# Fahad021/DER-VET

Hardware: AMD Instinct MI355X
Metric: dispatch LP windows/sec (whole node, 8760h monthly windows); % HBM roofline (higher is better)
Workload: dtype f64

## Files before the change

### der-vet_amd/csrc/dvh_band.hip

```cpp
#include <stdio.h>
#include <stdlib.h>

#include <algorithm>
#include <type_traits>

#include "dvh_device.h"

namespace dvh {
namespace {

constexpr int kBandSteps = 768;
constexpr int kJMax = 4;
constexpr int kNeedsEll = -2;

__host__ __device__ constexpr size_t band_lds_doubles(int B, int S, bool ice, bool lc) {
  const int NW = B / kWave, NC = ice ? 5 : 3, NR = ice ? 4 : 2;
  const size_t SB = (size_t)S * B;
  return 2 * (size_t)(B + 1) + kJMax + (size_t)kNRed * (NW + 1) + 4 + (size_t)kJMax * B + (NC + NR) * SB +
         (lc ? 5 * SB : 0) + (ice ? 6 * SB : 0);
}
__host__ __device__ constexpr size_t band_ints_bytes(int B, int S) { return sizeof(int32_t) * (4 * (size_t)S * B + 4); }
__host__ __device__ constexpr size_t band_drow_bytes(int B, int S) { return align16(sizeof(int32_t) * (size_t)S * B); }
__host__ __device__ constexpr size_t band_lds_bytes(int B, int S, bool ice, bool lc) {
  const size_t d = align16(sizeof(double) * band_lds_doubles(B, S, ice, lc));
  return (lc ? d : d + align16(band_ints_bytes(B, S))) + band_drow_bytes(B, S);
}
static_assert(band_lds_bytes(kBandSteps / 3, 3, false, true) == 77328, "three-step battery form: two windows per CU");
static_assert(band_lds_bytes(kBandSteps, 1, false, false) == 84192, "one-step battery form");
static_assert(band_lds_bytes(kBandSteps, 1, true, false) == 145632, "ICE form");

template <bool ICE>
struct BandTune {
  static constexpr bool kkt_inline = !ICE;
  static constexpr bool kkt_prefetch = !ICE;
  static constexpr bool pin_kx = ICE;
  static constexpr bool uniform_check_scalars = ICE;
  static constexpr bool gate_rdx = !ICE;
};
constexpr int kTauWavePrio = 2;

struct ColKkt {
  double rd2, cx, bt;
};
struct ColKktX : ColKkt {
  double rdx;
};
__device__ __noinline__ ColKkt col_kkt_o(double kt, double cj, double loj, double hij, double xj, float fd) {
  const double id = (double)__builtin_amdgcn_rcpf(fd);
  const double rs = cj - kt;
  const bool fl = isfinite(loj), fh = isfinite(hij);
  const double lam = (fl && fh) ? rs : (fl ? fmax(rs, 0.0) : (fh ? fmin(rs, 0.0) : 0.0));
  const double rd = (rs - lam) * id;
  return {rd * rd, cj * xj, (fl ? loj * fmax(lam, 0.0) : 0.0) + (fh ? hij * fmin(lam, 0.0) : 0.0)};
}
__device__ __forceinline__ ColKktX col_kkt_x_i(double kt, double cj, double loj, double hij, double xj, float fd) {
  const double id = (double)__builtin_amdgcn_rcpf(fd);
  const double rs = cj - kt;
  const bool fl = isfinite(loj), fh = isfinite(hij);
  const double lam = (fl && fh) ? rs : (fl ? fmax(rs, 0.0) : (fh ? fmin(rs, 0.0) : 0.0));
  const double rd = (rs - lam) * id;
  ColKktX r;
  r.rd2 = rd * rd;
  r.cx = cj * xj;
  r.bt = (fl ? loj * fmax(lam, 0.0) : 0.0) + (fh ? hij * fmin(lam, 0.0) : 0.0);
  r.rdx = fabs(rd) * fabs(xj * (double)fd);
  return r;
}
struct RowKkt {
  double rp2, y2;
};
__device__ __forceinline__ RowKkt row_kkt_i(double kv, double qi, double yi, float fd, int ge) {
  const double dr = (double)fd, idr = (double)__builtin_amdgcn_rcpf(fd);
  double r = (qi - kv) * idr;
  if (ge) r = fmax(r, 0.0);
  return {r * r, (yi * dr) * (yi * dr)};
}
__device__ __noinline__ RowKkt row_kkt_o(double kv, double qi, double yi, float fd, int ge) {
  return row_kkt_i(kv, qi, yi, fd, ge);
}
template <bool INL>
__device__ __forceinline__ RowKkt row_kkt_fn(double kv, double qi, double yi, float fd, int ge) {
  if constexpr (INL) return row_kkt_i(kv, qi, yi, fd, ge);
  else return row_kkt_o(kv, qi, yi, fd, ge);
}

constexpr int kNeedsPlain = -3;
#ifndef DVH_BAND_PROBE
#define DVH_BAND_PROBE 0
#endif
__device__ __forceinline__ unsigned long long probe_clock() {
#if DVH_BAND_PROBE
  return __builtin_amdgcn_s_memtime();
#else
  return 0ull;
#endif
}
__device__ __forceinline__ double fma_clamp01(double a, double b, double c) {
  double r;
  asm("v_fma_f64 %0, %1, %2, %3 clamp" : "=v"(r) : "v"(a), "v"(b), "v"(c));
  return r;
}

template <bool ICE>
__device__ __forceinline__ double usc(double v) {
  return BandTune<ICE>::uniform_check_scalars ? uniform(v) : v;
}
template <bool ICE>
__device__ __forceinline__ double sgpr_fresh(double v) {
  if constexpr (BandTune<ICE>::uniform_check_scalars) asm volatile("" : "+s"(v));
  return v;
}
template <int B, int S, bool ICE, bool LC, int WPS, bool GATE, bool BOX>
__device__ __forceinline__ void band_window(const Batch& b, const Work& w, const Chunk& ch, const Opts& o, const int k_in,
                                            const int tid) {
  const int k = __builtin_amdgcn_readfirstlane(k_in);
  using Tune = BandTune<ICE>;
  constexpr int NW = B / kWave;
  constexpr int SB = S * B;
  constexpr int NC = ICE ? 5 : 3;
  constexpr int NR = ICE ? 4 : 2;
  extern __shared__ __attribute__((aligned(16))) unsigned char smem[];
  const int kl = k - ch.first;
  const WinOff W = uniform_win(win_offsets(b, ch, k));
  const int n = W.n, m = W.m, meq = W.meq;
  const int lane = tid & 63, wid = __builtin_amdgcn_readfirstlane(tid >> 6);
  double* scal = w.scal + (int64_t)kl * kScal;
  const int T = meq - 1, J = n - (ICE ? 5 : 3) * T, MI = m - meq;
  const int MD = ICE ? MI - 2 * T : MI;
  auto bail = [&]() {
    if (tid == 0) {
      b.istats[2 * k] = kNeedsEll;
      b.istats[2 * k + 1] = 0;
    }
  };
  if (n > kSmallMax || m > kSmallMax || T < 1 || T > SB || J < 0 || J > kJMax || MD < 0 || MD > T ||
      (J == 0 && MD > 0)) {
    bail();
    return;
  }
  const int CE = 3 * T + J, CO = 4 * T + J;
  double* XE = reinterpret_cast<double*>(smem);
  double* YS = XE + (B + 1);
  double* XT = YS + (B + 1);
  double* red = XT + kJMax;
  double* TP = red + kNRed * (NW + 1) + 4;
  double* XP = TP + kJMax * B;
  double* YP = XP + NC * SB;
  double* RO = YP + NR * SB;
  double* CQ = RO + (ICE ? 6 * SB : 0);
  static_assert(sizeof(double) * (NC + NR) * SB >= band_ints_bytes(B, S), "the ints fit the images");
  int32_t* dcm = LC ? reinterpret_cast<int32_t*>(XP)
                    : reinterpret_cast<int32_t*>(smem + align16(sizeof(double) * band_lds_doubles(B, S, ICE, LC)));
  int32_t* ice_a = dcm + SB;
  int32_t* ice_b = ice_a + SB;
  int32_t* ice_n = ice_b + SB;
  int32_t* flag = ice_n + SB;
  int32_t* DRL = reinterpret_cast<int32_t*>(smem + band_lds_bytes(B, S, ICE, LC) - band_drow_bytes(B, S));

  const int32_t* gkp = b.indptr + W.row;
  const int32_t* gkc = b.indices + W.nz;
  const double* gkv = b.data + W.nz;
  const double* craw = b.c + W.on;
  const double* lraw = b.l + W.on;
  const double* uraw = b.u + W.on;
  const double* qraw = b.q + W.om;
  double* dcv = w.dc + W.wn;
  double* drv = w.dr + W.wm;
  auto dcf = [&](int j) -> double { return dcv[j]; };
  auto drf = [&](int i) -> double { return drv[i]; };
  double* xo_g = b.x + W.on;
  double* yo_g = b.y + W.om;

  for (int u = tid; u < SB; u += B) {
    dcm[u] = -1;
    ice_a[u] = 0x7fffffff;
    ice_b[u] = -1;
    ice_n[u] = 0;
  }
  if (tid == 0) flag[0] = flag[1] = flag[2] = 0;
  __syncthreads();
  int bad = 0, crossed = 0, unboxed = 0;
  for (int j = tid; j < J; j += B) crossed |= lraw[3 * T + j] > uraw[3 * T + j];
  for (int r = tid; r <= T; r += B) {
    const int p0 = gkp[r], len = gkp[r + 1] - p0;
    if (r == 0) {
      bad |= !(len == 1 && gkc[p0] == 2 * T);
      continue;
    }
    const int t = r - 1;
    if (len != (r < T ? 4 : 3)) {
      bad = 1;
      continue;
    }
    unsigned seen = 0;
    for (int e = 0; e < len; ++e) {
      const int c = gkc[p0 + e];
      const int kind = c == t ? 0 : c == T + t ? 1 : c == 2 * T + t ? 2 : (r < T && c == 2 * T + t + 1) ? 3 : 4;
      if (kind == 4 || ((seen >> kind) & 1u)) bad = 1;
      seen |= 1u << kind;
    }
    bad |= lraw[t] != 0.0 || lraw[T + t] != 0.0;
    crossed |= lraw[t] > uraw[t] || lraw[T + t] > uraw[T + t] || lraw[2 * T + t] > uraw[2 * T + t];
    if (BOX) unboxed |= !(isfinite(uraw[t]) && isfinite(uraw[T + t]) && isfinite(lraw[2 * T + t]) && isfinite(uraw[2 * T + t]));
    if (ICE) {
      if (BOX) unboxed |= !(isfinite(uraw[CE + t]) && isfinite(uraw[CO + t]));
      bad |= lraw[CE + t] != 0.0 || lraw[CO + t] != 0.0;
      crossed |= lraw[CE + t] > uraw[CE + t] || lraw[CO + t] > uraw[CO + t];
    }
  }
  for (int i = meq + tid; i < m; i += B) {
    const int p0 = gkp[i], len = gkp[i + 1] - p0;
    if (ICE && len == 2) {
      int te = -1, to = -1;
      for (int e = 0; e < 2; ++e) {
        const int c = gkc[p0 + e];
        if (c >= CE && c < CE + T) te = c - CE;
        else if (c >= CO && c < CO + T) to = c - CO;
      }
      if (te < 0 || te != to) {
        bad = 1;
        continue;
      }
      atomicMin(&ice_a[te], i);
      atomicMax(&ice_b[te], i);
      atomicAdd(&ice_n[te], 1);
      continue;
    }
    if (len != (ICE ? 4 : 3)) {
      bad = 1;
      continue;
    }
    int tc = -1, td = -1, jj = -1, te = ICE ? -1 : -2;
    for (int e = 0; e < len; ++e) {
      const int c = gkc[p0 + e];
      if (c < T) {
        bad |= tc >= 0;
        tc = c;
      } else if (c < 2 * T) {
        bad |= td >= 0;
        td = c - T;
      } else if (c >= 3 * T && c < 3 * T + J) {
        bad |= jj >= 0;
        jj = c - 3 * T;
      } else if (ICE && c >= CE && c < CE + T) {
        bad |= te >= 0;
        te = c - CE;
      } else {
        bad = 1;
      }
    }
    if (tc < 0 || td != tc || jj < 0 || (ICE && te != tc)) {
      bad = 1;
      continue;
    }
    if (atomicCAS(&dcm[tc], -1, i * 8 + jj) != -1) bad = 1;
  }
  if (bad) flag[0] = 1;
  if (crossed) flag[1] = 1;
  if (unboxed) flag[2] = 1;
  __syncthreads();
  if (ICE)
    for (int u = tid; u < T; u += B)
      if (ice_n[u] != 2) flag[0] = 1;
  __syncthreads();
  if (flag[1] != 0) {
    if (tid == 0) {
      scal[0] = 0.0;
      scal[6] = 3.0;
      b.istats[2 * k] = 1;
      b.istats[2 * k + 1] = 0;
      for (int u = 0; u < 4; ++u) b.stats[4 * k + u] = u == 0 ? NAN : 0.0;
    }
    return;
  }
  if (flag[0] != 0) {
    bail();
    return;
  }
  auto bail_plain = [&]() {
    if (tid == 0) {
      b.istats[2 * k] = kNeedsPlain;
      b.istats[2 * k + 1] = 0;
    }
  };
  if (BOX && flag[2] != 0) {
    bail_plain();
    return;
  }

  const int t0 = S * tid;
  bool val[S];
  double x[S][NC], xa[S][NC], cc[S][3], hi[S][3];
  double loe[S];
  double ks[S][4];
  double kd[S][4];
  double ka[S][2], kb[S][2];
  double kp0 = 0.0;
  double y[S][NR], ya[S][NR], q[S][2];
  int drow[S], jt[S], ra[S], rb[S];
  auto col = [&](int s, int v) { return v < 3 ? v * T + t0 + s : (v == 3 ? CE : CO) + t0 + s; };
  auto ro = [&](int u, int s) -> double& { return RO[(u * S + s) * B + tid]; };
  auto cqa = [&](int u, int s) -> double& { return CQ[(u * S + s) * B + tid]; };
#pragma unroll
  for (int s = 0; s < S; ++s) {
    const int t = t0 + s;
    val[s] = t < T;
#pragma unroll
    for (int v = 0; v < NC; ++v) x[s][v] = xa[s][v] = 0.0;
#pragma unroll
    for (int v = 0; v < 3; ++v) cc[s][v] = hi[s][v] = 0.0;
#pragma unroll
    for (int r = 0; r < NR; ++r) y[s][r] = ya[s][r] = 0.0;
#pragma unroll
    for (int u = 0; u < 4; ++u) ks[s][u] = kd[s][u] = 0.0;
    ka[s][0] = ka[s][1] = kb[s][0] = kb[s][1] = 0.0;
    q[s][0] = q[s][1] = 0.0;
    loe[s] = 0.0;
    drow[s] = -1;
    DRL[s * B + tid] = -1;
    jt[s] = 0;
    ra[s] = rb[s] = -1;
    if (ICE)
      for (int u = 0; u < 6; ++u) ro(u, s) = 0.0;
    if (LC)
      for (int u = 0; u < 5; ++u) cqa(u, s) = 0.0;
  }
  auto cof = [&](int s, int v) -> double { return v < 3 ? (LC ? cqa(v, s) : cc[s][v]) : ro(v - 3, s); };
  auto qv = [&](int s, int r) -> double { return LC ? cqa(3 + r, s) : q[s][r]; };
  auto hib = [&](int s, int v) -> double { return v < 3 ? hi[s][v] : ro(v - 1, s); };
  auto rhs = [&](int s, int r) -> double { return r < 2 ? qv(s, r) : ro(r + 2, s); };
#pragma unroll
  for (int s = 0; s < S; ++s) {
    if (!val[s]) continue;
    const int t = t0 + s;
    for (int p = gkp[t + 1]; p < gkp[t + 2]; ++p) {
      const int c = gkc[p];
      const double a = gkv[p];
      if (c == t) ks[s][0] = a;
      else if (c == T + t) ks[s][1] = a;
      else if (c == 2 * T + t) ks[s][2] = a;
      else ks[s][3] = a;
    }
    if (s == 0)
      for (int p = gkp[t]; p < gkp[t + 1]; ++p)
        if (gkc[p] == 2 * T + t) kp0 = gkv[p];
    const int dv = dcm[t];
    if (dv >= 0) {
      drow[s] = dv >> 3;
      DRL[s * B + tid] = drow[s];
      jt[s] = dv & 7;
      for (int p = gkp[drow[s]]; p < gkp[drow[s] + 1]; ++p) {
        const int c = gkc[p];
        const double a = gkv[p];
        if (c < T) kd[s][0] = a;
        else if (c < 2 * T) kd[s][1] = a;
        else if (c < 3 * T + J) kd[s][2] = a;
        else kd[s][3] = a;
      }
    }
    if (ICE) {
      ra[s] = ice_a[t];
      rb[s] = ice_b[t];
      for (int p = gkp[ra[s]]; p < gkp[ra[s] + 1]; ++p) (gkc[p] < CO ? ka[s][0] : ka[s][1]) = gkv[p];
      for (int p = gkp[rb[s]]; p < gkp[rb[s] + 1]; ++p) (gkc[p] < CO ? kb[s][0] : kb[s][1]) = gkv[p];
    }
  }
  auto row_of = [&](int s, int r) -> int {
    return r == 0 ? (val[s] ? t0 + s + 1 : -1) : r == 1 ? drow[s] : (val[s] ? (r == 2 ? ra[s] : rb[s]) : -1);
  };
  constexpr int kInitLane = kWave - 1;
  static_assert(kJMax < kInitLane, "tau lanes and the init-row lane are distinct");
  const bool tlane = wid == 0 && lane < J, ilane = wid == 0 && lane == kInitLane;
  double sp[6] = {0.0, 0.0, 0.0, 0.0, 0.0, 0.0};

  double fcv[S][NC], frv[S][NR], fsp = 1.0, kin0 = 0.0;
#pragma unroll
  for (int s = 0; s < S; ++s) {
#pragma unroll
    for (int v = 0; v < NC; ++v) fcv[s][v] = 1.0;
#pragma unroll
    for (int r = 0; r < NR; ++r) frv[s][r] = 1.0;
  }
  if (ilane) kin0 = gkv[gkp[0]];
  auto factor = [](double a) { return a > 0.0 ? __builtin_amdgcn_rsq(a) : 1.0; };
  auto exchange = [&]() {
    XE[tid] = fcv[0][2];
    YS[tid + 1] = frv[S - 1][0];
    if (tid == 0) XE[B] = 1.0;
    if (tid < kJMax) XT[tid] = tlane ? fsp : 1.0;
    if (ilane) YS[0] = fsp;
  };
  for (int pass = 0; pass <= o.ruiz_iters; ++pass) {
    const bool pc = pass == o.ruiz_iters;
    auto acc = [pc](double a, double v) { return pc ? a + v : fmax(a, v); };
    exchange();
    __syncthreads();
    const double fen = XE[tid + 1], frp = YS[tid];
    double nr[S][NR], nc[S][NC];
#pragma unroll
    for (int s = 0; s < S; ++s) {
      const double fe1 = s < S - 1 ? fcv[s < S - 1 ? s + 1 : s][2] : fen;
      const double rp = s == 0 ? frp : frv[s > 0 ? s - 1 : 0][0];
      const double kpr = s == 0 ? kp0 : ks[s > 0 ? s - 1 : 0][3];
      const double r0 = frv[s][0], r1 = frv[s][1], ftj = XT[jt[s]];
      nr[s][0] = acc(acc(acc(fabs(ks[s][0]) * r0 * fcv[s][0], fabs(ks[s][1]) * r0 * fcv[s][1]),
                         fabs(ks[s][2]) * r0 * fcv[s][2]),
                     fabs(ks[s][3]) * r0 * fe1);
      nr[s][1] = acc(acc(fabs(kd[s][0]) * r1 * fcv[s][0], fabs(kd[s][1]) * r1 * fcv[s][1]), fabs(kd[s][2]) * r1 * ftj);
      nc[s][0] = acc(fabs(ks[s][0]) * r0 * fcv[s][0], fabs(kd[s][0]) * r1 * fcv[s][0]);
      nc[s][1] = acc(fabs(ks[s][1]) * r0 * fcv[s][1], fabs(kd[s][1]) * r1 * fcv[s][1]);
      nc[s][2] = acc(fabs(kpr) * rp * fcv[s][2], fabs(ks[s][2]) * r0 * fcv[s][2]);
      if constexpr (ICE) {
        const double r2 = frv[s][NR > 2 ? 2 : 0], r3 = frv[s][NR > 3 ? 3 : 0];
        const double f3 = fcv[s][NC > 3 ? 3 : 0], f4 = fcv[s][NC > 4 ? 4 : 0];
        nr[s][1] = acc(nr[s][1], fabs(kd[s][3]) * r1 * f3);
        nr[s][NR > 2 ? 2 : 0] = acc(fabs(ka[s][0]) * r2 * f3, fabs(ka[s][1]) * r2 * f4);
        nr[s][NR > 3 ? 3 : 0] = acc(fabs(kb[s][0]) * r3 * f3, fabs(kb[s][1]) * r3 * f4);
        nc[s][NC > 3 ? 3 : 0] = acc(acc(fabs(kd[s][3]) * r1 * f3, fabs(ka[s][0]) * r2 * f3), fabs(kb[s][0]) * r3 * f3);
        nc[s][NC > 4 ? 4 : 0] = acc(fabs(ka[s][1]) * r2 * f4, fabs(kb[s][1]) * r3 * f4);
      }
    }
    for (int j = 0; j < J; ++j) {
      const double ftj = XT[j];
      double a = 0.0;
#pragma unroll
      for (int s = 0; s < S; ++s)
        if (jt[s] == j) a = acc(a, fabs(kd[s][2]) * frv[s][1] * ftj);
      TP[j * B + tid] = a;
    }
    double nsp = 0.0;
    if (ilane) nsp = fabs(kin0) * fsp * XE[0];
    __syncthreads();
    if (wid == 0) {
      for (int j = 0; j < J; ++j) {
        double a = TP[j * B + lane];
#pragma unroll
        for (int r = 1; r < NW; ++r) a = acc(a, TP[j * B + r * kWave + lane]);
        a = uniform(pc ? wave_sum_dpp(a) : wave_max(a));
        if (lane == j) nsp = a;
      }
    }
#pragma unroll
    for (int s = 0; s < S; ++s) {
#pragma unroll
      for (int v = 0; v < NC; ++v) fcv[s][v] *= factor(nc[s][v]);
#pragma unroll
      for (int r = 0; r < NR; ++r) frv[s][r] *= factor(nr[s][r]);
    }
    if (tlane || ilane) fsp *= factor(nsp);
    __syncthreads();
  }
  {
    auto oor = [](double f) { return !(f >= 0x1p-100 && f <= 0x1p100); };
    bool out = oor(fsp);
#pragma unroll
    for (int s = 0; s < S; ++s) {
#pragma unroll
      for (int v = 0; v < NC; ++v) out |= oor(fcv[s][v]);
#pragma unroll
      for (int r = 0; r < NR; ++r) out |= oor(frv[s][r]);
    }
    if (__syncthreads_or(out)) {
      bail();
      return;
    }
  }
  exchange();
  __syncthreads();
  {
    const double fen = XE[tid + 1], frp = YS[tid];
    kp0 = kp0 * frp * fcv[0][2];
#pragma unroll
    for (int s = 0; s < S; ++s) {
      const double fe1 = s < S - 1 ? fcv[s < S - 1 ? s + 1 : s][2] : fen;
      const double r0 = frv[s][0], r1 = frv[s][1];
      ks[s][0] = ks[s][0] * r0 * fcv[s][0];
      ks[s][1] = ks[s][1] * r0 * fcv[s][1];
      ks[s][2] = ks[s][2] * r0 * fcv[s][2];
      ks[s][3] = ks[s][3] * r0 * fe1;
      kd[s][0] = kd[s][0] * r1 * fcv[s][0];
      kd[s][1] = kd[s][1] * r1 * fcv[s][1];
      kd[s][2] = kd[s][2] * r1 * XT[jt[s]];
      if constexpr (ICE) {
        const double r2 = frv[s][NR > 2 ? 2 : 0], r3 = frv[s][NR > 3 ? 3 : 0];
        const double f3 = fcv[s][NC > 3 ? 3 : 0], f4 = fcv[s][NC > 4 ? 4 : 0];
        kd[s][3] = kd[s][3] * r1 * f3;
        ka[s][0] = ka[s][0] * r2 * f3;
        ka[s][1] = ka[s][1] * r2 * f4;
        kb[s][0] = kb[s][0] * r3 * f3;
        kb[s][1] = kb[s][1] * r3 * f4;
      }
    }
    if (ilane) kin0 = kin0 * fsp * XE[0];
  }
  double nrm[4] = {0.0, 0.0, 0.0, 0.0};
#pragma unroll
  for (int s = 0; s < S; ++s) {
    if (!val[s]) continue;
    const int t = t0 + s;
#pragma unroll
    for (int v = 0; v < NC; ++v) {
      const int j = col(s, v);
      const double d = fcv[s][v], cj = craw[j];
      const double csj = cj * d, lsj = lraw[j] / d, usj = uraw[j] / d;
      if (v < 3) {
        hi[s][v] = usj;
        if (LC)
          cqa(v, s) = csj;
        else
          cc[s][v] = csj;
      } else {
        ro(v - 1, s) = usj;
        ro(v - 3, s) = csj;
      }
      if (v == 2) loe[s] = lsj;
      x[s][v] = xa[s][v] = fmin(fmax(o.warm ? xo_g[j] / d : 0.0, lsj), usj);
      nrm[0] += csj * csj;
      nrm[2] += cj * cj;
      dcv[j] = d;
      w.fc[W.wn + j] = (float)d;
    }
#pragma unroll
    for (int r = 0; r < NR; ++r) {
      const int i = row_of(s, r);
      if (i < 0) continue;
      const double d = frv[s][r], qi = qraw[i], qsi = qi * d;
      if (r == 0) {
        if (LC)
          cqa(3, s) = qsi;
        else
          q[s][0] = qsi;
      } else if (r == 1) {
        if (LC)
          cqa(4, s) = qsi;
        else
          q[s][1] = qsi;
      } else {
        ro(r + 2, s) = qsi;
      }
      if (o.warm) y[s][r] = ya[s][r] = r == 0 ? yo_g[i] / d : fmax(yo_g[i] / d, 0.0);
      nrm[1] += qsi * qsi;
      nrm[3] += qi * qi;
      drv[i] = d;
      w.fr[W.wm + i] = (float)d;
    }
  }
  if (tlane) {
    const int j = 3 * T + lane;
    const double cj = craw[j], l0 = lraw[j] / fsp, h0 = uraw[j] / fsp;
    sp[0] = sp[1] = sp[5] = fmin(fmax(o.warm ? xo_g[j] / fsp : 0.0, l0), h0);
    sp[2] = cj * fsp;
    sp[3] = l0;
    sp[4] = h0;
    nrm[0] += sp[2] * sp[2];
    nrm[2] += cj * cj;
    dcv[j] = fsp;
    w.fc[W.wn + j] = (float)fsp;
  }
  if (ilane) {
    const double q0 = qraw[0];
    sp[3] = q0 * fsp;
    sp[4] = kin0;
    if (o.warm) sp[0] = sp[1] = sp[2] = yo_g[0] / fsp;
    nrm[1] += sp[3] * sp[3];
    nrm[3] += q0 * q0;
    drv[0] = fsp;
    w.fr[W.wm] = (float)fsp;
  }
  block_sum<B, 4>(nrm, red);
  const double ncs = sqrt(nrm[0]), nqs = sqrt(nrm[1]);
  const double pw0 = (ncs > 1e-10 && nqs > 1e-10) ? ncs / nqs : 1.0;
  int xta[S];
#pragma unroll
  for (int s = 0; s < S; ++s) xta[s] = lds_addr(XT + jt[s]);
  if constexpr (LC) __syncthreads();
  auto xpi = [&](int v, int s) -> double& { return XP[(v * S + s) * B + tid]; };
  auto ypi = [&](int r, int s) -> double& { return YP[(r * S + s) * B + tid]; };
  if (tid < kJMax) XT[tid] = 0.0;
  if (tid == 0) XE[B] = YS[B] = 0.0;
  XE[tid] = YS[tid] = 0.0;
  for (int u = tid; u < kJMax * B; u += B) TP[u] = 0.0;
#pragma unroll
  for (int s = 0; s < S; ++s) {
#pragma unroll
    for (int v = 0; v < NC; ++v) xpi(v, s) = x[s][v];
#pragma unroll
    for (int r = 0; r < NR; ++r) ypi(r, s) = y[s][r];
  }
  __syncthreads();

  auto kpv = [&](int s) { return s == 0 ? kp0 : ks[s > 0 ? s - 1 : 0][3]; };
  auto ktr = [&](int s, const double (&vr)[NR], double vprev, double (&out)[NC]) {
    out[0] = fma(kd[s][0], vr[1], ks[s][0] * vr[0]);
    out[1] = fma(kd[s][1], vr[1], ks[s][1] * vr[0]);
    out[2] = fma(ks[s][2], vr[0], kpv(s) * vprev);
    if constexpr (ICE) {
      out[3] = fma(kb[s][0], vr[3], fma(ka[s][0], vr[2], kd[s][3] * vr[1]));
      out[4] = fma(kb[s][1], vr[3], ka[s][1] * vr[2]);
    }
  };
  auto kown = [&](int s, const double (&v)[NC], double (&os)[NR]) {
    os[0] = fma(ks[s][2], v[2], fma(ks[s][1], v[1], ks[s][0] * v[0]));
    os[1] = fma(kd[s][1], v[1], kd[s][0] * v[0]);
    if constexpr (ICE) {
      os[1] = fma(kd[s][3], v[3], os[1]);
      os[2] = fma(ka[s][1], v[4], ka[s][0] * v[3]);
      os[3] = fma(kb[s][1], v[4], kb[s][0] * v[3]);
    }
  };
  auto kfin_next = [&](int s, double (&os)[NR], double vnext) { os[0] = fma(ks[s][3], vnext, os[0]); };
  auto kfin_tau = [&](int s, double (&os)[NR]) { os[1] = fma(kd[s][2], lds_ld(xta[s]), os[1]); };
  auto ktr_c = [&](int s, const double (&vr)[NR], double vprev, double (&out)[NC]) {
    out[0] = fma(kd[s][0], vr[1], fma(ks[s][0], vr[0], -cof(s, 0)));
    out[1] = fma(kd[s][1], vr[1], fma(ks[s][1], vr[0], -cof(s, 1)));
    out[2] = fma(ks[s][2], vr[0], fma(kpv(s), vprev, -cof(s, 2)));
    if constexpr (ICE) {
      out[3] = fma(kb[s][0], vr[3], fma(ka[s][0], vr[2], fma(kd[s][3], vr[1], -cof(s, 3))));
      out[4] = fma(kb[s][1], vr[3], fma(ka[s][1], vr[2], -cof(s, 4)));
    }
  };
  auto kown_q = [&](int s, const double (&v)[NC], double (&os)[NR]) {
    os[0] = fma(ks[s][2], v[2], fma(ks[s][1], v[1], fma(ks[s][0], v[0], -qv(s, 0))));
    os[1] = fma(kd[s][1], v[1], fma(kd[s][0], v[0], -qv(s, 1)));
    if constexpr (ICE) {
      os[1] = fma(kd[s][3], v[3], os[1]);
      os[2] = fma(ka[s][1], v[4], fma(ka[s][0], v[3], -rhs(s, 2)));
      os[3] = fma(kb[s][1], v[4], fma(kb[s][0], v[3], -rhs(s, 3)));
    }
  };
  auto tau_parts = [&](const double (&vd)[S]) {
    if (J == 1) {
      double a = kd[0][2] * vd[0];
#pragma unroll
      for (int s = 1; s < S; ++s) a = fma(kd[s][2], vd[s], a);
      TP[tid] = a;
    } else {
      for (int j = 0; j < J; ++j) {
        double a = (jt[0] == j ? kd[0][2] : 0.0) * vd[0];
#pragma unroll
        for (int s = 1; s < S; ++s) a = fma(jt[s] == j ? kd[s][2] : 0.0, vd[s], a);
        TP[j * B + tid] = a;
      }
    }
  };
  auto tau_parts_of = [&](const double (&vr)[S][NR]) {
    double vd[S];
#pragma unroll
    for (int s = 0; s < S; ++s) vd[s] = vr[s][1];
    tau_parts(vd);
  };
  auto tau_kt = [&]() {
    double res = 0.0;
// ... 10 lines not shown
  double eta = o.step_safety;
  if (o.power_iters > 0) {
    const int P = o.power_iters;
    const double v0 = 1.0 / sqrt((double)n);
    double vc[S][NC];
#pragma unroll
    for (int s = 0; s < S; ++s)
#pragma unroll
      for (int v = 0; v < NC; ++v) vc[s][v] = val[s] ? v0 : 0.0;
    double vtau = (wid == 0 && lane < J) ? v0 : 0.0;
    double nv[2] = {0.0, 0.0};
    double wr[S][NR];
#pragma unroll
    for (int s = 0; s < S; ++s)
#pragma unroll
      for (int r = 0; r < NR; ++r) wr[s][r] = 0.0;
    for (int pi = 0; pi <= P; ++pi) {
      if (pi > 0) {
        const double ysp = YS[tid];
#pragma unroll
        for (int s = 0; s < S; ++s) ktr(s, wr[s], s == 0 ? ysp : wr[s > 0 ? s - 1 : 0][0], vc[s]);
        if (wid == 0) {
          const double kt = tau_kt();
          vtau = lane < J ? kt : 0.0;
        }
      }
      if (pi >= P - 1) {
        double a = vtau * vtau;
#pragma unroll
        for (int s = 0; s < S; ++s)
#pragma unroll
          for (int v = 0; v < NC; ++v) a = fma(vc[s][v], vc[s][v], a);
        nv[pi - (P - 1)] = a;
      }
      if (pi == P) break;
      XE[tid] = vc[0][2];
      if (wid == 0 && lane < J) XT[lane] = vtau;
      __syncthreads();
      const double xen = XE[tid + 1];
#pragma unroll
      for (int s = 0; s < S; ++s) {
        kown(s, vc[s], wr[s]);
        kfin_next(s, wr[s], s == S - 1 ? xen : vc[s < S - 1 ? s + 1 : s][2]);
        kfin_tau(s, wr[s]);
      }
      YS[tid + 1] = wr[S - 1][0];
      if (ilane) YS[0] = sp[4] * XE[0];
      tau_parts_of(wr);
      __syncthreads();
    }
    block_sum<B, 2>(nv, red);
    if (nv[0] > 0.0 && nv[1] > 0.0) eta = o.step_safety / sqrt(sqrt(nv[1] / nv[0]));
    YS[tid] = 0.0;
    if (tid == 0) YS[B] = 0.0;
    for (int u = tid; u < kJMax * B; u += B) TP[u] = 0.0;
    __syncthreads();
  }
  if (o.warm) {
    YS[tid + 1] = y[S - 1][0];
    if (ilane) YS[0] = sp[0];
    if (J > 0) tau_parts_of(y);
    __syncthreads();
  }
  eta = uniform(eta);
  double pwi = pw0;
  if (o.warm) {
    double nv[2] = {0.0, 0.0};
#pragma unroll
    for (int s = 0; s < S; ++s) {
#pragma unroll
      for (int v = 0; v < NC; ++v) nv[0] += x[s][v] * x[s][v];
#pragma unroll
      for (int r = 0; r < NR; ++r) nv[1] += y[s][r] * y[s][r];
    }
    if (tlane) nv[0] += sp[0] * sp[0];
    if (ilane) nv[1] += sp[0] * sp[0];
    block_sum<B, 2>(nv, red);
    if (nv[0] > 1e-20 && nv[1] > 1e-20) {
      const double ratio = sqrt(nv[1] / nv[0]);
      pwi = sqrt(ratio * pw0);
    }
  }
  double pw = uniform(pwi);
  double tj[S][3];
  double cbox = 0.0;
  if constexpr (BOX) {
    double wb[S][NC];
    bool unb = false;
#pragma unroll
    for (int s = 0; s < S; ++s) {
#pragma unroll
      for (int v = 0; v < NC; ++v) {
        double wv = hib(s, v) - (v == 2 ? loe[s] : 0.0);
        unb |= !isfinite(wv);
        if (!(wv >= 0x1p-500)) wv = 0.0;
        wb[s][v] = wv;
      }
    }
    if (__syncthreads_or(unb)) {
      bail_plain();
      return;
    }
    XP[tid] = wb[0][2];
    XP[B + 1 + tid] = loe[0];
    if (tid == 0) XP[B] = XP[2 * B + 1] = 0.0;
    __syncthreads();
    const double wnx = XP[tid + 1], lnx = XP[B + 2 + tid], we0 = XP[0], le0 = XP[B + 1];
    __syncthreads();
    double cl[1] = {0.0};
    kp0 *= wb[0][2];
#pragma unroll
    for (int s = 0; s < S; ++s) {
      const double wn1 = s < S - 1 ? wb[s < S - 1 ? s + 1 : s][2] : wnx;
      const double ln1 = s < S - 1 ? loe[s < S - 1 ? s + 1 : s] : lnx;
      if (val[s]) {
        const double qs = fma(-ks[s][3], ln1, fma(-ks[s][2], loe[s], qv(s, 0)));
        if (LC)
          cqa(3, s) = qs;
        else
          q[s][0] = qs;
        cl[0] = fma(cof(s, 2), loe[s], cl[0]);
      }
      ks[s][0] *= wb[s][0];
      ks[s][1] *= wb[s][1];
      ks[s][2] *= wb[s][2];
      ks[s][3] *= wn1;
      kd[s][0] *= wb[s][0];
      kd[s][1] *= wb[s][1];
      if constexpr (ICE) {
        const double we = wb[s][NC > 3 ? 3 : 0], wo = wb[s][NC > 4 ? 4 : 0];
        kd[s][3] *= we;
        ka[s][0] *= we;
        ka[s][1] *= wo;
        kb[s][0] *= we;
        kb[s][1] *= wo;
      }
#pragma unroll
      for (int v = 0; v < NC; ++v) {
        const double lo = v == 2 ? loe[s] : 0.0, wv = wb[s][v], cs = cof(s, v) * wv;
        if (v >= 3)
          ro(v - 3, s) = cs;
        else if (LC)
          cqa(v, s) = cs;
        else
          cc[s][v] = cs;
        const double xv = wv > 0.0 ? fmin(fmax((x[s][v] - lo) / wv, 0.0), 1.0) : 0.0;
        x[s][v] = xa[s][v] = xv;
        xpi(v, s) = xv;
        if (v < 3)
          tj[s][v < 3 ? v : 0] = wv > 0.0 ? uniform(eta / pw) / (wv * wv) : 0.0;
        else
          ro(v - 1, s) = wv > 0.0 ? uniform(eta / pw) / (wv * wv) : 0.0;
      }
    }
    if (ilane) {
      sp[3] = fma(-sp[4], le0, sp[3]);
      sp[4] *= we0;
    }
    block_sum<B, 1>(cl, red);
    cbox = cl[0];
  }
  const double cnorm = uniform(sqrt(nrm[2])), qnorm = uniform(sqrt(nrm[3])), c0 = uniform(b.c0[k] + cbox);
  int it = 0, kin = 0, status = kIterLimit;
  double r0 = -1.0, rprev = -1.0;
  double* fin = red + kNRed * NW;
  if (tid == 0)
// ... 139 lines not shown
      }
      XE[tid] = xb[0][2];
#pragma unroll
      for (int s = 0; s < S; ++s) {
        kown_q(s, xb[s], kx[s]);
        if (s < S - 1) kfin_next(s, kx[s], xb[s < S - 1 ? s + 1 : s][2]);
      }
      if constexpr (W0) {
        tau_update(uniform(wave_sum_dpp(ta0 + ta1)), ca, cb, chk_tag);
      } else {
        if (wid == 0 && J > 1) tau_update(tau_kt(), ca, cb, chk_tag);
      }
    }
    pstamp(0);
    if constexpr (!W0 && Tune::pin_kx) {
#pragma unroll
      for (int s = 0; s < S; ++s)
#pragma unroll
        for (int r = 0; r < NR; ++r) asm volatile("" ::"v"(kx[s][r]));
    }
    lds_barrier();
    if constexpr (W0) __builtin_amdgcn_s_setprio(0);
    pstamp(1);
    {
      const double xen = XE[tid + 1];
      double xtv[S];
#pragma unroll
      for (int s = 0; s < S; ++s) xtv[s] = lds_ld(xta[s]);
      kfin_next(S - 1, kx[S - 1], xen);
#pragma unroll
      for (int s = 0; s < S; ++s) {
        kx[s][1] = fma(kd[s][2], xtv[s], kx[s][1]);
#pragma unroll
        for (int r = 1; r < ((ICE && !W0) ? 2 : NR); ++r) row_step(s, r);
      }
      if (J > 0) tau_parts_of(y);
#pragma unroll
      for (int s = !W0 ? S - 1 : 0; s < S; ++s) row_step(s, 0);
      YS[tid + 1] = y[S - 1][0];
      if (W0 || wid == 0) {
        if (ilane) {
          const double y0 = sp[0], ya0 = sp[1];
          const double q1 = fma(sigma, sp[3] - sp[4] * XE[0], y0);
          if (CHECK) {
            const double d = y0 - q1, da = q1 - ya0;
            mv2 += d * d;
            mv3 += da * da;
            sp[2] = q1;
          }
          const double yn = fma(ca, fma(2.0, q1, -y0), cb * ya0);
          sp[0] = yn;
          YS[0] = yn;
        }
      }
    }
    ++it;
    ++kin;
    pstamp(2);
    if constexpr (W0) {
#pragma unroll
      for (int s = 0; s < S; ++s) {
#pragma unroll
        for (int v = 0; v < NC; ++v) asm volatile("" ::"v"(x[s][v]));
#pragma unroll
        for (int r = 0; r < NR; ++r) asm volatile("" ::"v"(y[s][r]));
      }
    }
    lds_barrier();
    if constexpr (!W0) {
#pragma unroll
      for (int s = 0; s < S - 1; ++s) row_step(s, 0);
    }
    if constexpr (ICE && !W0) {
#pragma unroll
      for (int s = 0; s < S; ++s)
#pragma unroll
        for (int r = 2; r < NR; ++r) row_step(s, r);
    }
    pstamp(3);
  };

  using F = std::integral_constant<bool, false>;
  using Tt = std::integral_constant<bool, true>;
  pstamp(-1);
  while (it < o.max_iters) {
    if (--ck != 0) {
      if (w0)
        iterate(F(), Tt());
      else
        iterate(F(), F());
      continue;
    }
    ck = chk;
    if (w0)
      iterate(Tt(), Tt());
    else
      iterate(Tt(), F());
    const bool last = it + chk > o.max_iters;
    bool kkt = (--kk_ == 0) || last;
    if (kkt) kk_ = kkt_every;
    static_assert(kRdx == kNRed - 1, "the dual-residual term is the last reduced value");
    constexpr int NRED = Tune::gate_rdx ? kNRed : kNRed - 1;
    double acc[NRED];
    acc[0] = fma(tau_bs, mvb0, mv0);
    acc[1] = fma(tau_bs, mvb1, mv1);
    acc[2] = mv2;
    acc[3] = mv3;
#pragma unroll
    for (int u = 4; u < NRED; ++u) acc[u] = 0.0;
    double r = 0.0;
    if constexpr (GATE) {
      double acc4[4] = {acc[0], acc[1], acc[2], acc[3]};
      block_sum1<B, 4, true>(acc4, red);
#pragma unroll
      for (int u = 0; u < 4; ++u) acc[u] = acc4[u];
      r = usc<ICE>(sqrt(pw * acc[0] + acc[2] / pw));
      if (kkt && !last && kkt_gate_skip(o, gate, r)) {
        kkt = false;
        ++gate.skip;
      }
    }
    if (kkt) {
      float fcl[S][NC], frl[S][NR], fspl = 1.0f;
      if constexpr (Tune::kkt_prefetch) {
        const int to = S * opaque(tid);
        const float* fcw = w.fc + W.wn;
        const float* frw = w.fr + W.wm;
#pragma unroll
        for (int s = 0; s < S; ++s) {
          const bool vs = to + s < T;
#pragma unroll
          for (int v = 0; v < NC; ++v) {
            const int j = v < 3 ? v * T + to + s : (v == 3 ? CE : CO) + to + s;
            const float f = fcw[vs ? j : 0];
            fcl[s][v] = vs ? f : 1.0f;
          }
#pragma unroll
          for (int r = 0; r < NR; ++r) {
            const int i = r == 0 ? (vs ? to + s + 1 : -1) : r == 1 ? DRL[s * B + tid] : (vs ? (r == 2 ? ra[s] : rb[s]) : -1);
            const float f = frw[i >= 0 ? i : 0];
            frl[s][r] = i >= 0 ? f : 1.0f;
          }
        }
        const int lo_ = (to / S) & (kWave - 1);
        const float ft = fcw[tlane ? 3 * T + lo_ : 0], fi = frw[0];
        fspl = tlane ? ft : ilane ? fi : 1.0f;
      }
      double xp[S][NC], yp[S][NR];
      load_images(xp, yp);
      XE[tid] = xp[0][2];
      YS[tid + 1] = yp[S - 1][0];
      if (ilane) YS[0] = sp[2];
      if (tlane) XT[lane] = sp[5];
      if (J > 0) tau_parts_of(yp);
      lds_barrier();
      auto col_kkt = [&](int j, double kt, double cj, double loj, double hij, double xj, float fpre) {
        const float fd = Tune::kkt_prefetch ? fpre : w.fc[W.wn + opaque(j)];
        static_assert(Tune::gate_rdx == Tune::kkt_inline, "col_kkt_x_i is inlined only, col_kkt_o out of line only");
        if constexpr (Tune::gate_rdx) {
          const ColKktX r = col_kkt_x_i(kt, cj, loj, hij, xj, fd);
          acc[5] += r.rd2;
          acc[6] += r.cx;
          acc[8] += r.bt;
          acc[kRdx] += r.rdx;
        } else {
          const ColKkt r = col_kkt_o(kt, cj, loj, hij, xj, fd);
// ... 48 lines not shown
    }
    if constexpr (GATE) {
      if (kkt) {
        double acc6[NRED - 4];
#pragma unroll
        for (int u = 4; u < NRED; ++u) acc6[u - 4] = acc[u];
        block_sum1<B, NRED - 4, true>(acc6, red + 4 * NW);
#pragma unroll
        for (int u = 4; u < NRED; ++u) acc[u] = acc6[u - 4];
      }
    } else if (kkt) {
      block_sum1<B, NRED, true>(acc, red);
    } else {
      double acc4[4] = {acc[0], acc[1], acc[2], acc[3]};
      block_sum1<B, 4, true>(acc4, red);
#pragma unroll
      for (int u = 0; u < 4; ++u) acc[u] = acc4[u];
    }
    if constexpr (!GATE) r = usc<ICE>(sqrt(pw * acc[0] + acc[2] / pw));
    if (kkt) {
      const double pobj = usc<ICE>(acc[6] + c0), dobj = usc<ICE>(acc[7] + acc[8] + c0);
      const double pres = usc<ICE>(sqrt(acc[4]) / (1.0 + sgpr_fresh<ICE>(qnorm)));
      const double dres = usc<ICE>(sqrt(acc[5]) / (1.0 + sgpr_fresh<ICE>(cnorm)));
      const double gap = usc<ICE>(fabs(pobj - dobj) / (1.0 + fabs(pobj) + fabs(dobj)));
      if (tid == 0) {
        fin[0] = pobj;
        fin[1] = pres;
        fin[2] = dres;
        fin[3] = gap;
      }
      if (kkt_done(o, pres, dres, gap, pobj, dobj, acc[4], acc[9], Tune::gate_rdx ? acc[kRdx] : 0.0)) {
        status = kOptimal;
        break;
      }
      if constexpr (GATE) {
        gate.note(pres, dres, gap, o.eps, r);
        gate.q = usc<ICE>(gate.q);
      }
      if (!(isfinite(pobj) && isfinite(dobj))) {
        status = kNumerical;
        break;
      }
    }
    if (r0 < 0.0) r0 = r;
    const bool restart = (r <= o.b_suff * r0) || (r <= o.b_nec * r0 && rprev >= 0.0 && r > rprev) ||
                         ((double)kin >= o.b_art * (double)it);
    if (restart) {
      const double ddx = sqrt(acc[1]), ddy = sqrt(acc[3]);
      if (ddx > 1e-10 && ddy > 1e-10) pw = uniform(pw_update<!ICE>(ddy / ddx, pw, o.theta));
      tau = uniform(eta / pw);
      sigma = uniform(eta * pw);
      sigma2n = uniform(-2.0 * sigma);
      box_steps_rescale();
      double xp[S][NC], yp[S][NR];
      load_images(xp, yp);
#pragma unroll
      for (int s = 0; s < S; ++s) {
#pragma unroll
        for (int v = 0; v < NC; ++v) {
          x[s][v] = xa[s][v] = xp[s][v];
        }
#pragma unroll
        for (int rr = 0; rr < NR; ++rr) {
          y[s][rr] = ya[s][rr] = yp[s][rr];
        }
      }
      if (ilane) sp[0] = sp[1] = sp[2];
      if (tlane) sp[0] = sp[1] = sp[5];
      kin = 0;
      kbase = 0;
      hw = hload(0);
      r0 = r;
      rprev = -1.0;
    } else {
      rprev = r;
    }
    if (restart || kkt) {
      YS[tid + 1] = y[S - 1][0];
      if (ilane) YS[0] = sp[0];
      if (J > 0) tau_parts_of(y);
      lds_barrier();
    }
  }
#pragma unroll
  for (int s = 0; s < S; ++s) {
    if (!val[s]) continue;
    const int t = t0 + s;
#pragma unroll
    for (int v = 0; v < NC; ++v) {
      const int j = col(s, v);
      if constexpr (BOX) {
        const double d = dcf(j), lo = lraw[j] / d, hv = uraw[j] / d;
        double wv = hv - (v == 2 ? lo : 0.0);
        if (!(wv >= 0x1p-500)) wv = 0.0;
        xo_g[j] = fmin(fmax(fma(wv, xpi(v, s), lo), lo), hv) * d;
      } else {
        xo_g[j] = xpi(v, s) * dcf(j);
      }
    }
    yo_g[t + 1] = ypi(0, s) * drf(t + 1);
    const int dr_ = DRL[s * B + tid];
    if (dr_ >= 0) yo_g[dr_] = ypi(1, s) * drf(dr_);
    if (ICE) {
      yo_g[ra[s]] = ypi(2, s) * drf(ra[s]);
      yo_g[rb[s]] = ypi(3, s) * drf(rb[s]);
    }
  }
  if (tlane) xo_g[3 * T + lane] = sp[5] * dcf(3 * T + lane);
  if (ilane) yo_g[0] = sp[2] * drf(0);
  if constexpr (DVH_BAND_PROBE) {
    pstamp(4);
    pacc[4] += (unsigned)(pt1 - pt2);
    unsigned hw = 0;
    asm volatile("s_getreg_b32 %0, hwreg(HW_REG_HW_ID)" : "=s"(hw));
    __syncthreads();
    if (lane == 0) {
      for (int u = 0; u < 5; ++u) xo_g[6 * wid + u] = (double)pacc[u];
      xo_g[6 * wid + 5] = (double)hw;
    }
  }
  if (tid == 0) {
    b.istats[2 * k] = status;
    b.istats[2 * k + 1] = it;
    for (int u = 0; u < 4; ++u) b.stats[4 * k + u] = fin[u];
  }
}

struct BandArgs {
  Batch b;
  Work w;
  Chunk ch;
  Opts o;
  const int32_t* list;
  int count;
  int32_t* queue;
};
template <int B, int S, bool ICE, bool LC, int WPS, bool GATE, bool BOX, bool PERSIST>
__global__ __launch_bounds__(B, WPS) void pdhg_band_kernel(const BandArgs args) {
  if constexpr (!PERSIST) {
    const int i = blockIdx.x;
    band_window<B, S, ICE, LC, WPS, GATE, BOX>(args.b, args.w, args.ch, args.o,
                                               args.list ? args.list[i] : args.ch.first + i, threadIdx.x);
  } else {
    __shared__ int32_t next;
    for (;;) {
#if defined(__HIP_DEVICE_COMPILE__)
      using KArgs = const __attribute__((address_space(4))) BandArgs*;
      KArgs kp = (KArgs)__builtin_amdgcn_kernarg_segment_ptr();
      asm volatile("" : "+s"(kp));
      const BandArgs& args = *(const BandArgs*)kp;
#endif
      if (__builtin_amdgcn_readfirstlane(threadIdx.x) < kWave)
        next = __builtin_amdgcn_readfirstlane(atomicAdd(args.queue, (threadIdx.x & (kWave - 1)) == 0 ? 1 : 0));
      __syncthreads();
      const int i = __builtin_amdgcn_readfirstlane(next);
      __syncthreads();
      if (i >= args.count) return;
      int tid = threadIdx.x;
#if defined(__HIP_DEVICE_COMPILE__)
      asm volatile("" : "+v"(tid));
#endif
      band_window<B, S, ICE, LC, WPS, GATE, BOX>(args.b, args.w, args.ch, args.o,
                                                 args.list ? args.list[i] : args.ch.first + i, tid);
    }
  }
}

template <int B, int S, bool ICE, bool LC, int WPS, bool GATE, bool BOX, bool PERSIST>
hipError_t launch_band_one_q(const Batch& b, const Work& w, const Chunk& ch, const Opts& o, hipStream_t s,
                             const int32_t* list, int nlist, int* variant_out) {
  static_assert(B * S == kBandSteps, "every form covers T <= kBandSteps");
  const size_t lds = band_lds_bytes(B, S, ICE, LC);
  auto kern = pdhg_band_kernel<B, S, ICE, LC, WPS, GATE, BOX, PERSIST>;
  hipError_t e = hipFuncSetAttribute((const void*)kern, hipFuncAttributeMaxDynamicSharedMemorySize, (int)lds);
  if (e != hipSuccess) return e;
  if (getenv("DVH_BAND_OCC")) {
    int nb = -1, dev = 0;
    hipGetDevice(&dev);
    hipDeviceProp_t pr;
    hipGetDeviceProperties(&pr, dev);
    hipOccupancyMaxActiveBlocksPerMultiprocessor(&nb, (const void*)kern, B, lds);
    hipFuncAttributes fa;
    hipFuncGetAttributes(&fa, (const void*)kern);
    fprintf(stderr, "band<%d,%d,%d,%d,gate %d,box %d,persist %d>: lds %zu B, blocks/CU %d, lds/CU %zu, regs %d, local %zu\n",
            B, S, (int)ICE, (int)LC, (int)GATE, (int)BOX, (int)PERSIST, lds, nb, (size_t)pr.maxSharedMemoryPerMultiProcessor,
            fa.numRegs, (size_t)fa.localSizeBytes);
  }
  const int count = list ? nlist : ch.count;
  if (count <= 0) return hipSuccess;
  int grid = count;
  if (PERSIST) {
    int& slots = w.slots[(ICE ? 4 : 0) + (GATE ? 2 : 0) + (BOX ? 1 : 0)];
    if (slots <= 0) {
      int nb = 0, cus = 0, dev = 0;
      if ((e = hipGetDevice(&dev)) != hipSuccess) return e;
      if ((e = hipOccupancyMaxActiveBlocksPerMultiprocessor(&nb, (const void*)kern, B, lds)) != hipSuccess) return e;
      if ((e = hipDeviceGetAttribute(&cus, hipDeviceAttributeMultiprocessorCount, dev)) != hipSuccess) return e;
      slots = std::max(1, nb) * std::max(1, cus);
    }
    static const int reserve = [] { const char* e = getenv("DVH_BAND_RESERVE"); return e ? std::max(0, atoi(e)) : 0; }();
    grid = std::min(count, std::max(1, slots - 2 * reserve));
    if ((e = hipMemsetAsync(w.queue, 0, sizeof(int32_t), s)) != hipSuccess) return e;
// ... 73 lines not shown
```

Before: 305,700.

## Batch setup loads and write-back in the three-step battery band kernel

For the non-ICE, three-step, box-bounded band form, the structure check now reads row pointers, column indices and bounds up front and records whether rows are in canonical sorted order. When they are, the KKT coefficients are gathered with straight-line indexed loads instead of per-row CSR loops. Warm-start and rhs loads are hoisted into per-step batches, and the final write-back loads its scale and bound values before storing. The goal is more independent global loads in flight during setup and teardown, at the cost of more registers. It also adds probe-only segment timers.

```diff
diff --git a/der-vet_amd/csrc/dvh_band.hip b/der-vet_amd/csrc/dvh_band.hip
--- a/der-vet_amd/csrc/dvh_band.hip
+++ b/der-vet_amd/csrc/dvh_band.hip
@@ -29,6 +29,9 @@
 static_assert(band_lds_bytes(kBandSteps, 1, false, false) == 84192, "one-step battery form");
 static_assert(band_lds_bytes(kBandSteps, 1, true, false) == 145632, "ICE form");
 
+#ifndef DVH_BAND_SETUP_BATCH
+#define DVH_BAND_SETUP_BATCH 1
+#endif
 template <bool ICE>
 struct BandTune {
   static constexpr bool kkt_inline = !ICE;
@@ -36,6 +39,8 @@
   static constexpr bool pin_kx = ICE;
   static constexpr bool uniform_check_scalars = ICE;
   static constexpr bool gate_rdx = !ICE;
+  template <int S, bool BOX>
+  static constexpr bool setup_batch = !ICE && S == 3 && BOX && DVH_BAND_SETUP_BATCH;
 };
 constexpr int kTauWavePrio = 2;
 
@@ -115,6 +120,15 @@
                                             const int tid) {
   const int k = __builtin_amdgcn_readfirstlane(k_in);
   using Tune = BandTune<ICE>;
+  unsigned fseg[7] = {0u, 0u, 0u, 0u, 0u, 0u, 0u};
+  unsigned long long ft = probe_clock();
+  auto fstamp = [&](int seg) __attribute__((always_inline)) {
+    if constexpr (DVH_BAND_PROBE) {
+      const unsigned long long t = probe_clock();
+      if (seg >= 0) fseg[seg] += (unsigned)(t - ft);
+      ft = t;
+    }
+  };
   constexpr int NW = B / kWave;
   constexpr int SB = S * B;
   constexpr int NC = ICE ? 5 : 3;
@@ -177,11 +191,81 @@
     ice_b[u] = -1;
     ice_n[u] = 0;
   }
+  constexpr bool kBatch = Tune::template setup_batch<S, BOX>;
   if (tid == 0) flag[0] = flag[1] = flag[2] = 0;
+  if constexpr (kBatch)
+    if (tid == 0) flag[3] = 0;
   __syncthreads();
   int bad = 0, crossed = 0, unboxed = 0;
   for (int j = tid; j < J; j += B) crossed |= lraw[3 * T + j] > uraw[3 * T + j];
-  for (int r = tid; r <= T; r += B) {
+  if constexpr (kBatch) {
+    static_assert(!kBatch || !ICE, "the batched structure check has no ICE rows");
+    int unsorted = 0;
+    for (int r = tid; r <= T; r += B) {
+      const int t = r > 0 ? r - 1 : 0;
+      const int p0 = gkp[r], p1 = gkp[r + 1];
+      const double l0 = lraw[t], l1 = lraw[T + t], l2 = lraw[2 * T + t];
+      const double u0 = uraw[t], u1 = uraw[T + t], u2 = uraw[2 * T + t];
+      const int len = p1 - p0, want = r == 0 ? 1 : r < T ? 4 : 3;
+      int c[4] = {-1, -1, -1, -1};
+      if (len == want) {
+#pragma unroll
+        for (int e = 0; e < 4; ++e) c[e] = gkc[p0 + (e < want ? e : 0)];
+      }
+      if (r == 0) {
+        bad |= !(len == 1 && c[0] == 2 * T);
+        continue;
+      }
+      if (len != want) {
+        bad = 1;
+        continue;
+      }
+      unsigned seen = 0;
+#pragma unroll
+      for (int e = 0; e < 4; ++e) {
+        if (e >= want) continue;
+        const int kind = c[e] == t ? 0 : c[e] == T + t ? 1 : c[e] == 2 * T + t ? 2 : (r < T && c[e] == 2 * T + t + 1) ? 3 : 4;
+        if (kind == 4 || ((seen >> kind) & 1u)) bad = 1;
+        seen |= 1u << kind;
+      }
+      unsorted |= !(c[0] == t && c[1] == T + t && c[2] == 2 * T + t && (r == T || c[3] == 2 * T + t + 1));
+      bad |= l0 != 0.0 || l1 != 0.0;
+      crossed |= l0 > u0 || l1 > u1 || l2 > u2;
+      if (BOX) unboxed |= !(isfinite(u0) && isfinite(u1) && isfinite(l2) && isfinite(u2));
+    }
+    for (int i = meq + tid; i < m; i += B) {
+      const int p0 = gkp[i], len = gkp[i + 1] - p0;
+      if (len != 3) {
+        bad = 1;
+        continue;
+      }
+      const int c[3] = {gkc[p0], gkc[p0 + 1], gkc[p0 + 2]};
+      int tc = -1, td = -1, jj = -1;
+#pragma unroll
+      for (int e = 0; e < 3; ++e) {
+        if (c[e] < T) {
+          bad |= tc >= 0;
+          tc = c[e];
+        } else if (c[e] < 2 * T) {
+          bad |= td >= 0;
+          td = c[e] - T;
+        } else if (c[e] >= 3 * T && c[e] < 3 * T + J) {
+          bad |= jj >= 0;
+          jj = c[e] - 3 * T;
+        } else {
+          bad = 1;
+        }
+      }
+      if (tc < 0 || td != tc || jj < 0) {
+        bad = 1;
+        continue;
+      }
+      unsorted |= !(c[0] < c[1] && c[1] < c[2]);
+      if (atomicCAS(&dcm[tc], -1, i * 8 + jj) != -1) bad = 1;
+    }
+    if (unsorted) flag[3] = 1;
+  }
+  for (int r = tid; !kBatch && r <= T; r += B) {
     const int p0 = gkp[r], len = gkp[r + 1] - p0;
     if (r == 0) {
       bad |= !(len == 1 && gkc[p0] == 2 * T);
@@ -208,7 +292,7 @@
       crossed |= lraw[CE + t] > uraw[CE + t] || lraw[CO + t] > uraw[CO + t];
     }
   }
-  for (int i = meq + tid; i < m; i += B) {
+  for (int i = meq + tid; !kBatch && i < m; i += B) {
     const int p0 = gkp[i], len = gkp[i + 1] - p0;
     if (ICE && len == 2) {
       int te = -1, to = -1;
@@ -287,6 +371,9 @@
     bail_plain();
     return;
   }
+  bool sorted = false;
+  if constexpr (kBatch) sorted = __builtin_amdgcn_readfirstlane(flag[3]) == 0;
+  fstamp(0);
 
   const int t0 = S * tid;
   bool val[S];
@@ -329,9 +416,46 @@
   auto qv = [&](int s, int r) -> double { return LC ? cqa(3 + r, s) : q[s][r]; };
   auto hib = [&](int s, int v) -> double { return v < 3 ? hi[s][v] : ro(v - 1, s); };
   auto rhs = [&](int s, int r) -> double { return r < 2 ? qv(s, r) : ro(r + 2, s); };
+  if (kBatch && sorted) {
+    int pr[S], pd[S], dvs[S];
+#pragma unroll
+    for (int s = 0; s < S; ++s) {
+      dvs[s] = val[s] ? dcm[t0 + s] : -1;
+      pr[s] = gkp[val[s] ? t0 + s + 1 : 0];
+    }
+    const int pz = gkp[val[0] ? t0 : 0];
+#pragma unroll
+    for (int s = 0; s < S; ++s) pd[s] = gkp[dvs[s] >= 0 ? dvs[s] >> 3 : 0];
+    double as[S][4], ad[S][3];
+#pragma unroll
+    for (int s = 0; s < S; ++s) {
+      const int p = val[s] ? pr[s] : 0, pq = dvs[s] >= 0 ? pd[s] : 0;
+#pragma unroll
+      for (int u = 0; u < 3; ++u) {
+        as[s][u] = gkv[p + u];
+        ad[s][u] = gkv[pq + u];
+      }
+      as[s][3] = gkv[t0 + s + 1 < T ? p + 3 : 0];
+    }
+    const double az = gkv[val[0] ? pz + (t0 == 0 ? 0 : 3) : 0];
+    kp0 = val[0] ? az : 0.0;
+#pragma unroll
+    for (int s = 0; s < S; ++s) {
+      const bool has = dvs[s] >= 0;
+#pragma unroll
+      for (int u = 0; u < 3; ++u) {
+        ks[s][u] = val[s] ? as[s][u] : 0.0;
+        kd[s][u] = has ? ad[s][u] : 0.0;
+      }
+      ks[s][3] = t0 + s + 1 < T ? as[s][3] : 0.0;
+      drow[s] = has ? dvs[s] >> 3 : -1;
+      DRL[s * B + tid] = drow[s];
+      jt[s] = has ? dvs[s] & 7 : 0;
+    }
+  }
 #pragma unroll
   for (int s = 0; s < S; ++s) {
-    if (!val[s]) continue;
+    if (!val[s] || (kBatch && sorted)) continue;
     const int t = t0 + s;
     for (int p = gkp[t + 1]; p < gkp[t + 2]; ++p) {
       const int c = gkc[p];
@@ -365,6 +489,7 @@
       for (int p = gkp[rb[s]]; p < gkp[rb[s] + 1]; ++p) (gkc[p] < CO ? kb[s][0] : kb[s][1]) = gkv[p];
     }
   }
+  fstamp(1);
   auto row_of = [&](int s, int r) -> int {
     return r == 0 ? (val[s] ? t0 + s + 1 : -1) : r == 1 ? drow[s] : (val[s] ? (r == 2 ? ra[s] : rb[s]) : -1);
   };
@@ -493,9 +618,31 @@
     }
     if (ilane) kin0 = kin0 * fsp * XE[0];
   }
+  fstamp(2);
   double nrm[4] = {0.0, 0.0, 0.0, 0.0};
+  double bx[NC], bq[NR], by[NR];
+  auto step_loads = [&](int s) __attribute__((always_inline)) {
+#pragma unroll
+    for (int r = 0; r < NR; ++r) {
+      const int i = row_of(s, r);
+      bq[r] = qraw[i < 0 ? 0 : i];
+      by[r] = 0.0;
+    }
+#pragma unroll
+    for (int v = 0; v < NC; ++v) bx[v] = 0.0;
+    if (o.warm) {
+#pragma unroll
+      for (int v = 0; v < NC; ++v) bx[v] = xo_g[val[s] ? col(s, v) : 0];
+#pragma unroll
+      for (int r = 0; r < NR; ++r) {
+        const int i = row_of(s, r);
+        by[r] = yo_g[i < 0 ? 0 : i];
+      }
+    }
+  };
 #pragma unroll
   for (int s = 0; s < S; ++s) {
+    if constexpr (kBatch) step_loads(s);
     if (!val[s]) continue;
     const int t = t0 + s;
 #pragma unroll
@@ -514,7 +661,7 @@
         ro(v - 3, s) = csj;
       }
       if (v == 2) loe[s] = lsj;
-      x[s][v] = xa[s][v] = fmin(fmax(o.warm ? xo_g[j] / d : 0.0, lsj), usj);
+      x[s][v] = xa[s][v] = fmin(fmax(o.warm ? (kBatch ? bx : xo_g)[kBatch ? v : j] / d : 0.0, lsj), usj);
       nrm[0] += csj * csj;
       nrm[2] += cj * cj;
       dcv[j] = d;
@@ -524,7 +671,7 @@
     for (int r = 0; r < NR; ++r) {
       const int i = row_of(s, r);
       if (i < 0) continue;
-      const double d = frv[s][r], qi = qraw[i], qsi = qi * d;
+      const double d = frv[s][r], qi = (kBatch ? bq : qraw)[kBatch ? r : i], qsi = qi * d;
       if (r == 0) {
         if (LC)
           cqa(3, s) = qsi;
@@ -538,7 +685,7 @@
       } else {
         ro(r + 2, s) = qsi;
       }
-      if (o.warm) y[s][r] = ya[s][r] = r == 0 ? yo_g[i] / d : fmax(yo_g[i] / d, 0.0);
+      if (o.warm) y[s][r] = ya[s][r] = r == 0 ? (kBatch ? by : yo_g)[kBatch ? r : i] / d : fmax((kBatch ? by : yo_g)[kBatch ? r : i] / d, 0.0);
       nrm[1] += qsi * qsi;
       nrm[3] += qi * qi;
       drv[i] = d;
@@ -568,6 +715,7 @@
     w.fr[W.wm] = (float)fsp;
   }
   block_sum<B, 4>(nrm, red);
+  fstamp(3);
   const double ncs = sqrt(nrm[0]), nqs = sqrt(nrm[1]);
   const double pw0 = (ncs > 1e-10 && nqs > 1e-10) ? ncs / nqs : 1.0;
   int xta[S];
@@ -744,6 +892,7 @@
     }
   }
   double pw = uniform(pwi);
+  fstamp(4);
   double tj[S][3];
   double cbox = 0.0;
   if constexpr (BOX) {
@@ -1049,6 +1198,7 @@
 
   using F = std::integral_constant<bool, false>;
   using Tt = std::integral_constant<bool, true>;
+  fstamp(5);
   pstamp(-1);
   while (it < o.max_iters) {
     if (--ck != 0) {
@@ -1263,8 +1413,35 @@
       lds_barrier();
     }
   }
-#pragma unroll
-  for (int s = 0; s < S; ++s) {
+  fstamp(-1);
+  if constexpr (kBatch) {
+    static_assert(!kBatch || (BOX && !ICE), "the batched write-back is the battery box form's");
+#pragma unroll
+    for (int s = 0; s < S; ++s) {
+      double wd[NC], wl[NC], wu[NC];
+      const int dr_ = DRL[s * B + tid];
+#pragma unroll
+      for (int v = 0; v < NC; ++v) {
+        const int j = val[s] ? col(s, v) : 0;
+        wd[v] = dcf(j);
+        wl[v] = lraw[j];
+        wu[v] = uraw[j];
+      }
+      const double wr0 = drf(val[s] ? t0 + s + 1 : 0), wr1 = drf(dr_ >= 0 ? dr_ : 0);
+      if (!val[s]) continue;
+#pragma unroll
+      for (int v = 0; v < NC; ++v) {
+        const double d = wd[v], lo = wl[v] / d, hv = wu[v] / d;
+        double wv = hv - (v == 2 ? lo : 0.0);
+        if (!(wv >= 0x1p-500)) wv = 0.0;
+        xo_g[col(s, v)] = fmin(fmax(fma(wv, xpi(v, s), lo), lo), hv) * d;
+      }
+      yo_g[t0 + s + 1] = ypi(0, s) * wr0;
+      if (dr_ >= 0) yo_g[dr_] = ypi(1, s) * wr1;
+    }
+  }
+#pragma unroll
+  for (int s = 0; !kBatch && s < S; ++s) {
     if (!val[s]) continue;
     const int t = t0 + s;
 #pragma unroll
@@ -1290,6 +1467,7 @@
   if (tlane) xo_g[3 * T + lane] = sp[5] * dcf(3 * T + lane);
   if (ilane) yo_g[0] = sp[2] * drf(0);
   if constexpr (DVH_BAND_PROBE) {
+    fstamp(6);
     pstamp(4);
     pacc[4] += (unsigned)(pt1 - pt2);
     unsigned hw = 0;
@@ -1299,6 +1477,8 @@
       for (int u = 0; u < 5; ++u) xo_g[6 * wid + u] = (double)pacc[u];
       xo_g[6 * wid + 5] = (double)hw;
     }
+    if (tid == 0)
+      for (int u = 0; u < 7; ++u) xo_g[6 * NW + u] = (double)fseg[u];
   }
   if (tid == 0) {
     b.istats[2 * k] = status;
```

Measured after the change: 306,700 (median of 6 runs). No clear change (+0.3%).
